# AugmentariumLab/VolumeRenderer

Measured on AMD Instinct MI355X. Metric: Mvoxels/s kd-tree compress+decode, higher is better.
Workload: dtype u8; 1 GPU; 2048x2048x1920 uint8 volume per GPU as 960 bricks of 256x256x128, rm_volume, tolerance 1, maxEpochs 2, VolumeKdtree build + levelCut

## Files before the change

volumerenderer_amd/csrc/brickset.h:

```cpp
#pragma once
#include "kd_common.h"
#include "../../include/vrhip.h"
#include <algorithm>
#include <string>
#include <vector>

namespace vr {

struct Stream2 {
    uint8_t *temp = nullptr;
    uint8_t *codes = nullptr;
    uint8_t *recon[3] = {nullptr, nullptr, nullptr};
    Ctrl *ctrl = nullptr;
    uint8_t *tree = nullptr;
    uint8_t *treeCompact = nullptr;
};

#define EST_R0_BUDGET 8
struct Switches {
    bool decodeWalk = false;
    bool decodeFineV1 = false;
    bool decodeQuad = false;
    bool noSkipBlocks = false;
    bool noUniformBlocks = false;
    bool estExactBounds = false;
    int estBudget = EST_R0_BUDGET;
    bool pyramidBoxes = false;
    bool indexPerBlock = false;
    bool noUniformDecode = false;
};

#define VR_LOD_SLOTS 4
struct LodSlot {
    int32_t *dev = nullptr;
    int32_t *host = nullptr;
    uint8_t *idxValCut = nullptr;
    uint32_t *decTables = nullptr;
    uint8_t *rankVals = nullptr;
    int64_t *obDev = nullptr;
    int64_t *obHost = nullptr;
    vr_pool_entry *tabHost = nullptr;
    int64_t tabCap = 0;
    hipEvent_t done = nullptr;
    bool pending = false;
};

struct BrickSet {
    int32_t B = 0;
    Switches sw;
    Geom g{};
    TilePlan tile{};
    RegionPlan region{};
    Pyr12Plan pyr12{};
    int32_t D = 0, maxDepth = 0;
    int32_t tolerance = 6, maxEpochs = 5, variant = 0;
    int32_t K = 0;
    int32_t Ds = 0;
    int64_t heapStride = 0;
    int64_t leafStride = 0;
    int64_t codeStride = 0;
    int64_t reconStride = 0;
    bool leafless = false;
    int64_t treeCap = 0;
    int64_t nIdx = 0;

    Stream2 mid, rng;
    uint8_t *mmMin[2] = {nullptr, nullptr}, *mmMax[2] = {nullptr, nullptr};
    unsigned long long *blockErr = nullptr;
    int64_t nErrBlk = 0;
    void *estSumm = nullptr;
    int64_t estSummStride = 0;
    unsigned long long *blockL1 = nullptr;
    uint8_t *blockFlag = nullptr;
    uint8_t *blockFlagR = nullptr;
    uint8_t *blockAlive = nullptr, *blockVal = nullptr;
    unsigned long long *blockSpine = nullptr, *blockSpineR = nullptr;
    uint32_t *chainLut = nullptr;
    uint32_t *blockTot = nullptr, *blockOff = nullptr;
    bool idx64 = false;
    unsigned long long *blockOff64 = nullptr, *idxBase = nullptr;
    int64_t nEmitBlk = 0;
// ... 80 lines not shown
```

volumerenderer_amd/csrc/capi.hip:

```cpp
#include "../../include/vrhip.h"
#include "brickset.h"
#include "raymarch.h"
#include <math.h>
#include <stdio.h>
#include <stdlib.h>
#include <string.h>
#include <algorithm>
#include <array>
#include <atomic>
#include <map>
#include <mutex>
#include <new>

using namespace vr;

struct vr_brickset { BrickSet s; };

#define HIPCHK(x) do { hipError_t e_ = (x); if (e_ != hipSuccess) return e_ == hipErrorOutOfMemory ? VR_ERR_OOM : VR_ERR_NO_DEVICE; } while (0)

static bool device_ok()
{
    int n = 0;
    hipError_t e = hipGetDeviceCount(&n);
    if ((e != hipSuccess || n <= 0) && getenv("VRHIP_DEBUG"))
// ... 160 lines not shown
    const vr_status rc = alloc_encoder_buffers(b);
    if (rc != VR_OK) { (void)hipGetLastError(); free_encoder_buffers(b); return rc; }
    b.encoderReady = true;
    return VR_OK;
}

vr_status vr_brickset_destroy(vr_brickset *h)
{
    if (!h) return VR_OK;
    BrickSet &b = h->s;
    free_lod_slots(&b);
    hipFree(b.errTable);
    free_encoder_buffers(b);
    free_stream2(b.mid);
    free_stream2(b.rng);
    hipFree(b.brickOff); hipFree(b.compactOverflow);
    hipFree(b.idxOff); hipFree(b.idxVal); hipFree(b.idxValCut); hipFree(b.fineIdx); hipFree(b.idxVal3); hipFree(b.boxUniform); hipFree(b.chainTab); hipFree(b.decTables); hipFree(b.lut); hipFree(b.spread); hipFree(b.srcIdx); hipFree(b.ownerRank); hipFree(b.ownerSurv); hipFree(b.rankVals);
    for (int i = 0; i < 8; ++i) if (b.ev[i]) hipEventDestroy(b.ev[i]);
    if (b.evFork) hipEventDestroy(b.evFork);
    for (int i = 0; i < 3; ++i) { if (b.evJoinN[i]) hipEventDestroy(b.evJoinN[i]); if (b.auxN[i]) hipStreamDestroy(b.auxN[i]); }
    delete h;
    return VR_OK;
}

static bool pow2(int64_t v) { return v > 0 && (v & (v - 1)) == 0; }

static bool misaligned16(const void *p) { return ((uintptr_t)p & 15) != 0; }

vr_status vr_brickset_create(vr_brickset **out, int32_t num_bricks, const int64_t dims[3], int32_t tolerance,
                             int32_t max_epochs, int32_t variant)
{
    if (!out || !dims || num_bricks <= 0) return VR_ERR_INVALID;
    if (tolerance < 0 || max_epochs < 0 || variant < 0 || variant > 2) return VR_ERR_INVALID;
    for (int k = 0; k < 3; ++k) if (dims[k] <= 0) return VR_ERR_INVALID;
    if (max_epochs > VR_MAX_EPOCHS) return VR_ERR_UNSUPPORTED;
    bool general = !pow2(dims[0]) || !pow2(dims[1]) || !pow2(dims[2]) || dims[0] > 1024 || dims[1] > 1024 || dims[2] > 1024;
    if (dims[0] > (1ll << 20) || dims[1] > (1ll << 20) || dims[2] > (1ll << 20) || dims[0] * dims[1] * dims[2] >= (1ll << 32))
        return VR_ERR_UNSUPPORTED;
    if (!device_ok()) return VR_ERR_NO_DEVICE;
    vr_brickset *h = new (std::nothrow) vr_brickset();
    if (!h) return VR_ERR_OOM;
    BrickSet &b = h->s;
    b.B = num_bricks;
    {
        Switches &w = b.sw;
        w.decodeWalk = getenv("VRHIP_DECODE_WALK") != nullptr;
        w.decodeFineV1 = getenv("VRHIP_DECODE_FINE_V1") != nullptr;
        w.decodeQuad = getenv("VRHIP_DECODE_QUAD") != nullptr;
        w.noSkipBlocks = getenv("VRHIP_NO_SKIP_BLOCKS") != nullptr;
        w.noUniformBlocks = getenv("VRHIP_NO_UNIFORM_BLOCKS") != nullptr;
        w.noUniformDecode = getenv("VRHIP_NO_UNIFORM_DECODE") != nullptr;
        w.pyramidBoxes = getenv("VRHIP_PYRAMID_BOXES") != nullptr;
        w.indexPerBlock = getenv("VRHIP_INDEX_PER_BLOCK") != nullptr;
        w.estExactBounds = getenv("VRHIP_EST_EXACT_BOUNDS") != nullptr;
        if (const char *eb = getenv("VRHIP_EST_BUDGET")) { const int v = atoi(eb); if (v >= 0) w.estBudget = v; }
    }
    make_geom(b.g, dims);
    b.D = b.g.D;
    if (b.D > 31) { delete h; return VR_ERR_UNSUPPORTED; }
    b.idx64 = b.D > 28 || (getenv("VRHIP_FORCE_IDX64") && b.D >= 12);
    if (b.idx64) general = true;
    if (b.idx64 && num_bricks != 1 && b.D > 28) { delete h; return VR_ERR_UNSUPPORTED; }
    b.generalGeom = general;
    b.maxDepth = b.D + VR_CHAIN_LEVELS;
    b.tolerance = tolerance; b.maxEpochs = max_epochs; b.variant = variant;
    b.K = b.D < 6 ? b.D : 6;
    b.Ds = b.D - b.K;
    b.heapStride = (int64_t)1 << (b.D + 1);
    b.leafStride = (int64_t)1 << b.D;
    b.codeStride = ((b.heapStride + 15) / 16) * 4;
    b.reconStride = b.leafStride;
    const int64_t numMax = b.heapStride - 1 + VR_CHAIN_LEVELS * b.leafStride;
    b.treeCap = ((numMax + 15) / 16 + 2) * 4 + 256;
    if (b.D >= 12) {
        const int64_t gappedBytes = ((int64_t)1 << (b.D - 12)) * 2320 * 4 + 256;
        if (gappedBytes > b.treeCap) b.treeCap = gappedBytes;
    }
    b.nIdx = (int64_t)1 << b.Ds;
    make_plans(b.g, b.K, b.generalGeom, b.idx64, b.treeCap, b.tile, b.region, b.pyr12);
    vr_status rc = alloc_stream2(b, b.mid);
    if (rc == VR_OK) {
        hipError_t e = hipMalloc(&b.idxOff, (size_t)b.B * b.nIdx * sizeof(uint32_t));
        if (e == hipSuccess) e = hipMalloc(&b.idxVal, (size_t)b.B * b.nIdx);
        if (e == hipSuccess) e = hipMalloc(&b.idxValCut, (size_t)b.B * b.nIdx);
        if (e == hipSuccess && general) {
            const int grc = build_general_geometry(&b);
            if (grc != 0) e = grc == -3 ? hipErrorOutOfMemory : hipErrorUnknown;
        }
        const auto upload = [](uint32_t *dst, const std::vector<uint32_t> &v) {
            return hipMemcpy(dst, v.data(), v.size() * sizeof(uint32_t), hipMemcpyHostToDevice);
        };
        if (e == hipSuccess) e = hipMalloc(&b.lut, ((size_t)1 << b.K) * sizeof(uint32_t));
        if (e == hipSuccess && !general) e = upload(b.lut, make_lut(b.g, b.K));
        if (e == hipSuccess && !general) e = hipMalloc(&b.spread, (size_t)(b.g.X + b.g.Y + b.g.Z) * sizeof(uint32_t));
        if (e == hipSuccess && !general) e = upload(b.spread, make_spread(b.g));
        for (int i = 0; i < 8 && e == hipSuccess; ++i) e = hipEventCreate(&b.ev[i]);
        if (e != hipSuccess) rc = e == hipErrorOutOfMemory ? VR_ERR_OOM : VR_ERR_NO_DEVICE;
    }
    if (rc != VR_OK) { vr_brickset_destroy(h); return rc; }
    b.hostCtrl.resize(b.B);
    b.openTreeBytes.assign(b.B, -1);
    *out = h;
    return VR_OK;
}

vr_status vr_brickset_set_switch(vr_brickset *h, const char *name, int32_t value)
{
    if (!h || !name) return VR_ERR_INVALID;
    Switches &w = h->s.sw;
    const bool on = value != 0;
    if (!strcmp(name, "decode_walk")) w.decodeWalk = on;
    else if (!strcmp(name, "decode_fine_v1")) w.decodeFineV1 = on;
    else if (!strcmp(name, "decode_quad")) w.decodeQuad = on;
    else if (!strcmp(name, "no_skip_blocks")) w.noSkipBlocks = on;
    else if (!strcmp(name, "no_uniform_blocks")) w.noUniformBlocks = on;
    else if (!strcmp(name, "no_uniform_decode")) w.noUniformDecode = on;
    else if (!strcmp(name, "pyramid_boxes")) w.pyramidBoxes = on;
    else if (!strcmp(name, "index_per_block")) w.indexPerBlock = on;
    else if (!strcmp(name, "est_exact_bounds")) w.estExactBounds = on;
    else return VR_ERR_INVALID;
    return VR_OK;
}

vr_status vr_brickset_set_compaction(vr_brickset *h, int32_t on_build)
{
    if (!h) return VR_ERR_INVALID;
    h->s.compactOnBuild = on_build != 0;
    return VR_OK;
}

vr_status vr_debug_set(const char *name, int32_t value)
{
    if (!name) return VR_ERR_INVALID;
    if (!strcmp(name, "skip_grid_v1")) { vr::g_skipGridV1.store(value ? 1 : 0); return VR_OK; }
    if (!strcmp(name, "reslice_tile_w")) {
        if (value != 8 && value != 16 && value != 64) return VR_ERR_INVALID;
        vr::g_resliceTileLog2.store(value == 8 ? 3 : (value == 16 ? 4 : 6));
        return VR_OK;
    }
    if (!strcmp(name, "hist_plain")) { vr::g_histPlain.store(value ? 1 : 0); return VR_OK; }
    return VR_ERR_INVALID;
}

vr_status vr_brickset_set_error_tolerance(vr_brickset *h, int32_t tol)
{
    if (!h || tol < 0) return VR_ERR_INVALID;
    h->s.tolerance = tol;
    return VR_OK;
}
vr_status vr_brickset_set_max_epochs(vr_brickset *h, int32_t e)
{
    if (!h || e < 0) return VR_ERR_INVALID;
    if (e > VR_MAX_EPOCHS) return VR_ERR_UNSUPPORTED;
    h->s.maxEpochs = e;
    return VR_OK;
}

vr_status vr_brickset_build(vr_brickset *h, const uint8_t *vox, void *stream)
{
    if (!h || !vox) return VR_ERR_INVALID;
    BrickSet &b = h->s;
    if (build_loads_vectors(&b) && misaligned16(vox)) return VR_ERR_INVALID;
    if (b.encoderReady && b.leafless != leafless_build(b)) {
        HIPCHK(hipDeviceSynchronize());
        free_encoder_buffers(b);
    }
    vr_status rc = ensure_encoder_buffers(b);
    if (rc != VR_OK) return rc;
    b.hostCtrlValid = false;
    b.hostBrickOff.clear();
    b.foreign = false;
// ... 1059 lines not shown
```

volumerenderer_amd/csrc/kd_encode.hip:

```cpp
#include "brickset.h"
#include <math.h>
#include <stdio.h>
#include <stdlib.h>
#include <string.h>

namespace vr {

#define FILL_NODES_PER_BLOCK 1024
#define EMIT_RANKS_PER_BLOCK 256

template <bool FROM_VOXELS>
__global__ void __launch_bounds__(256)
k_pyramid(Geom g, int dLeaf, int L, const uint8_t *__restrict__ vox, const uint8_t *__restrict__ inMin,
          const uint8_t *__restrict__ inMax, int64_t inStride, uint8_t *__restrict__ temp, int64_t heapStride,
          uint8_t *__restrict__ tempRange, uint8_t *__restrict__ outMin, uint8_t *__restrict__ outMax,
          int64_t outStride, const uint32_t *__restrict__ srcIdx)
{
    __shared__ uint8_t smn[2][1024], smx[2][1024];
    const int brick = blockIdx.y;
    const uint32_t n = 1u << L;
    const uint32_t base = blockIdx.x << L;
    uint8_t *T = temp + (int64_t)brick * heapStride;
    uint8_t *TR = tempRange ? tempRange + (int64_t)brick * heapStride : nullptr;
    for (uint32_t i = threadIdx.x; i < n; i += blockDim.x) {
// ... 2439 lines not shown
            if (b < nb && deadS[b]) { const uint32_t v4 = (uint32_t)valS[b] * 0x01010101u; pVal[t] = make_uint4(v4, v4, v4, v4); }
        }
#pragma unroll
        for (int k = 0; k < IDX_BLOCKS / 8; ++k) {
            const uint32_t p = (uint32_t)t + 256u * k, b = p >> 5;
            if (b < nb && deadS[b]) { const uint32_t v4 = (uint32_t)valS[b] * 0x01010101u; pVal3[p] = make_uint4(v4, v4, v4, v4); }
        }
    }
    if (w >= nLive) return;
    int dist[10];
#pragma unroll
    for (int i = 0; i < 10; ++i) dist[i] = __builtin_amdgcn_readfirstlane((int)distS[i]);
    if (D == 12) dist[0] = 0;
    const auto entry = [&](const IdxLoads &L, uint32_t b) {
        const uint32_t blk = blk0 + b;
        int val = idx_step(valS[b], rootS[b], dist[0]);
        uint32_t code6 = 0;
#pragma unroll
        for (int q = 1; q < 7; ++q) {
            code6 = L.cb[q] >> ((idx_off(idx_first(D, blk, q), lane, q) & 3u) * 2u);
            val = idx_step(val, code6, dist[q]);
        }
        const uint32_t c5 = L.c5 >> ((lane & 1u) * 4u);
        const bool root3 = (code6 & 3u) == 3u;
        const int64_t io = io0 + ((int64_t)blk << 6) + lane;
        a.idxOff[io] = (L.local != VR_IDX_DEAD && !root3) ? (a.idxBase ? 0u : blk * (uint32_t)PE_TOKENS) + L.local : VR_IDX_DEAD;
        a.idxVal[io] = (uint8_t)val;
        int v5[2], v4[4];
        uint32_t lo3 = 0, hi3 = 0;
#pragma unroll
        for (int i = 0; i < 2; ++i) v5[i] = idx_step(val, c5 >> (2 * i), dist[7]);
#pragma unroll
        for (int i = 0; i < 4; ++i) v4[i] = idx_step(v5[i >> 1], L.c4 >> (2 * i), dist[8]);
#pragma unroll
        for (int i = 0; i < 8; ++i) {
            const uint32_t v = (uint32_t)idx_step(v4[i >> 1], L.c3 >> (2 * i), dist[9]);
            if (i < 4) lo3 |= v << (8 * i); else hi3 |= v << (8 * (i - 4));
        }
        *(uint2 *)(a.idxVal3 + io * 8) = make_uint2(lo3, hi3);
    };
    const auto block_of = [&](uint32_t e) { return (uint32_t)__builtin_amdgcn_readfirstlane((int)listS[e]); };
    for (uint32_t e = w; e < nLive; e += 8u) {
        const uint32_t e1 = e + 4u < nLive ? e + 4u : e;
        const IdxLoads oth = idx_loads(a, Cb, io0, blk0 + block_of(e1), lane);
        entry(cur, block_of(e));
        if (e1 == e) break;
        const uint32_t e2 = e + 8u < nLive ? e + 8u : e1;
        cur = idx_loads(a, Cb, io0, blk0 + block_of(e2), lane);
        entry(oth, block_of(e1));
    }
}

#define CC_BLOCKS 16
#define CC_BATCH 4
template <bool RANGE>
__global__ void __launch_bounds__(256)
k_concat12(EmitArgs a, const uint8_t *__restrict__ gap, int64_t nblk)
{
    __shared__ unsigned long long g0S[CC_BLOCKS], spineS[CC_BLOCKS];
    __shared__ uint32_t totS[CC_BLOCKS], cntS[CC_BLOCKS];
    __shared__ unsigned long long bwIdx[2 * CC_BLOCKS];
    __shared__ uint32_t bwVal[2 * CC_BLOCKS];
    __shared__ uint32_t chunkPre[CC_BLOCKS + 1];
    __shared__ uint8_t chunkBlk[CC_BLOCKS * (PE_WORDS / 4 + 4)];
    const int brick = blockIdx.y, t = threadIdx.x;
    Ctrl &c = a.ctrls[brick];
    if (c.constBrick) return;
    if (a.brickOff && a.brickOff[gridDim.y] > (unsigned long long)a.compactCap) return;
    const int64_t blk0 = (int64_t)blockIdx.x * CC_BLOCKS;
    const int64_t base = a.brickOff ? (int64_t)a.brickOff[brick] : (int64_t)brick * a.treeCap;
    uint32_t *G0 = (uint32_t *)((RANGE ? a.treeR : a.tree) + base);
    const uint64_t capTok = a.brickOff ? ~0ull >> 2 : (uint64_t)a.treeCap * 4ull;
    if (t < 2 * CC_BLOCKS) { bwIdx[t] = ~0ull; bwVal[t] = 0u; }
    if (t < CC_BLOCKS) {
        const int64_t blk = blk0 + t;
        unsigned long long g0 = 0, sp = 0;
        uint32_t tot = 0, cnt = 0;
        if (blk < nblk) {
            const int64_t bo = (int64_t)brick * a.nEmitBlk + blk;
            const int bflags = a.blockAlive[bo];
            sp = RANGE ? a.blockSpineR[bo] : a.blockSpine[bo];
            g0 = a.blockOff64 ? a.blockOff64[bo] : (unsigned long long)a.blockOff[bo];
            tot = (bflags & 1) ? a.blockTot[bo] : 0u;
            cnt = (bflags & 2) && tot ? tot - (uint32_t)(sp >> 56) : 0u;
            if (tot && g0 + tot + 32ull > capTok) { atomicMax(&c.emitOverflow, 1); tot = 0; cnt = 0; }
        }
        g0S[t] = g0; spineS[t] = sp; totS[t] = tot; cntS[t] = cnt;
    }
    __syncthreads();
    if (t < CC_BLOCKS && totS[t] != 0u && totS[t] <= 32u) {
        const unsigned long long g0 = g0S[t];
        const uint32_t tot = totS[t], cnt = cntS[t];
        const int nsp = (int)(spineS[t] >> 56);
        unsigned long long v = spineS[t] & 0x00FFFFFFFFFFFFFFull;
        if (cnt) {
            const uint32_t *slot = (const uint32_t *)(gap + (int64_t)brick * a.treeCap) + (size_t)(blk0 + t) * PE_WORDS;
            unsigned long long sv = slot[0];
            if (cnt > 16u) sv |= (unsigned long long)slot[1] << 32;
            if (cnt < 32u) sv &= (1ull << (2 * cnt)) - 1ull;
            v |= sv << (2 * nsp);
        }
        const uint32_t sh = (uint32_t)(g0 & 15ull) * 2u;
        const uint64_t w0 = g0 >> 4, wl = (g0 + tot - 1) >> 4;
        const uint32_t x0 = (uint32_t)(v << sh), x1 = (uint32_t)((v << sh) >> 32), x2 = sh ? (uint32_t)(v >> (64u - sh)) : 0u;
        bwIdx[2 * t] = w0; bwVal[2 * t] = x0;
        if (wl == w0 + 1) { bwIdx[2 * t + 1] = wl; bwVal[2 * t + 1] = x1; }
        else if (wl == w0 + 2) { G0[w0 + 1] = x1; bwIdx[2 * t + 1] = wl; bwVal[2 * t + 1] = x2; }
    }
    if (t == 0) {
        uint32_t run = 0;
        for (int i = 0; i < CC_BLOCKS; ++i) {
            chunkPre[i] = run;
            if (totS[i] > 32u) {
                const uint64_t w0 = g0S[i] >> 4, wl = (g0S[i] + totS[i] - 1) >> 4;
                run += (uint32_t)((wl - (w0 & ~3ull)) / 4 + 1);
            }
        }
        chunkPre[CC_BLOCKS] = run;
    }
    __syncthreads();
    const uint32_t nchunkAll = chunkPre[CC_BLOCKS];
    for (int i = 0; i < CC_BLOCKS; ++i)
        for (uint32_t j = chunkPre[i] + (uint32_t)t; j < chunkPre[i + 1]; j += 256u) chunkBlk[j] = (uint8_t)i;
    __syncthreads();
    const uint32_t *gapW = (const uint32_t *)(gap + (int64_t)brick * a.treeCap) + (size_t)blk0 * PE_WORDS;
    for (uint32_t j0 = (uint32_t)t; j0 < nchunkAll; j0 += 256u * CC_BATCH) {
        uint32_t sv[CC_BATCH][5];
#pragma unroll
        for (int k = 0; k < CC_BATCH; ++k) {
            const uint32_t j = j0 + 256u * (uint32_t)k;
#pragma unroll
            for (int m = 0; m < 5; ++m) sv[k][m] = 0u;
            if (j >= nchunkAll) continue;
            const int i = chunkBlk[j];
            const unsigned long long g0 = g0S[i];
            const uint32_t cnt = cntS[i];
            const int nsp = (int)(spineS[i] >> 56);
            const int nws = (int)((cnt + 15u) >> 4);
            const uint32_t *slot = gapW + (size_t)i * PE_WORDS;
            const uint64_t wA = (g0 >> 4) & ~3ull;
            const long long so = 2ll * ((long long)(16ull * wA) - (long long)g0 - nsp) + 128ll * (long long)(j - chunkPre[i]);
            const int sw = (int)(so >> 5);
            if (cnt && sw >= 0 && sw + 4 < nws) {
                struct __attribute__((packed, aligned(4))) U4 { uint32_t x, y, z, w; };
                const U4 u = *(const U4 *)(slot + sw);
                sv[k][0] = u.x; sv[k][1] = u.y; sv[k][2] = u.z; sv[k][3] = u.w; sv[k][4] = slot[sw + 4];
            } else {
#pragma unroll
                for (int m = 0; m < 5; ++m) sv[k][m] = (cnt && sw + m >= 0 && sw + m < nws) ? slot[sw + m] : 0u;
            }
        }
#pragma unroll
        for (int k = 0; k < CC_BATCH; ++k) {
            const uint32_t j = j0 + 256u * (uint32_t)k;
            if (j >= nchunkAll) continue;
            const int i = chunkBlk[j];
            const unsigned long long g0 = g0S[i];
            const uint32_t tot = totS[i], cnt = cntS[i];
            const int nsp = (int)(spineS[i] >> 56);
            const unsigned long long spine = spineS[i] & 0x00FFFFFFFFFFFFFFull;
            const uint64_t w0 = g0 >> 4, wl = (g0 + tot - 1) >> 4;
            const uint64_t wA = w0 & ~3ull;
            const uint32_t q = j - chunkPre[i];
            const uint64_t d0 = wA + 4ull * (uint64_t)q;
            const long long so = 2ll * ((long long)(16ull * wA) - (long long)g0 - nsp) + 128ll * (long long)q;
            const uint32_t shf = (uint32_t)(so & 31ll);
            uint32_t o[4];
            const int tok0 = (int)(so >> 1);
            const bool edge = tok0 < 0 || tok0 + 64 > (int)cnt;
#pragma unroll
            for (int m = 0; m < 4; ++m) {
                o[m] = __builtin_amdgcn_alignbit(sv[k][m + 1], sv[k][m], shf);
                if (edge) {
                    const int tokAt = tok0 + 16 * m;
                    if (tokAt + 16 > (int)cnt) {
                        const int keep = (int)cnt - tokAt;
                        o[m] = keep <= 0 ? 0u : (keep >= 16 ? o[m] : (o[m] & ((1u << (2 * keep)) - 1u)));
                    }
                    if (tokAt < 0 && nsp) {
                        const long long bo2 = 2ll * ((long long)(16ull * (d0 + m)) - (long long)g0);
                        o[m] |= bo2 >= 0 ? (bo2 < 64 ? (uint32_t)(spine >> bo2) : 0u) : (uint32_t)(spine << (-bo2));
                    }
                }
            }
            if (d0 > w0 && d0 + 3 < wl) {
                *(uint4 *)(G0 + d0) = make_uint4(o[0], o[1], o[2], o[3]);
            } else {
#pragma unroll
                for (int m = 0; m < 4; ++m) {
                    const uint64_t d = d0 + m;
                    if (d < w0 || d > wl) continue;
                    if (d == w0) { bwIdx[2 * i] = d; bwVal[2 * i] = o[m]; }
                    else if (d == wl) { bwIdx[2 * i + 1] = d; bwVal[2 * i + 1] = o[m]; }
                    else G0[d] = o[m];
                }
            }
        }
    }
    __syncthreads();
    if (t < 2 * CC_BLOCKS) {
        const unsigned long long w = bwIdx[t];
        if (w != ~0ull) {
            bool first = true;
            uint32_t v = 0;
            unsigned long long wFirst = ~0ull, wLast = 0;
            for (int j = 0; j < 2 * CC_BLOCKS; ++j) {
                const unsigned long long wj = bwIdx[j];
                if (wj == ~0ull) continue;
                if (wFirst == ~0ull) wFirst = wj;
                wLast = wj;
                if (wj == w) { v |= bwVal[j]; if (j < t) first = false; }
            }
            if (first) {
                if (w == wFirst || w == wLast) { if (v) atomicOr(&G0[w], v); }
                else G0[w] = v;
            }
        }
    }
}

__global__ void __launch_bounds__(1024)
k_emit_stats(EmitArgs a, int64_t nblk)
{
    __shared__ unsigned long long sh[16];
    const int brick = blockIdx.x;
    if (a.ctrls[brick].constBrick) return;
    unsigned long long v = 0;
    for (int64_t i = threadIdx.x; i < nblk; i += blockDim.x) v = stat_merge(v, a.blockL1[(int64_t)brick * a.nEmitBlk + i]);
    for (int o = 32; o > 0; o >>= 1) v = stat_merge(v, __shfl_xor(v, o));
    if ((threadIdx.x & 63) == 0) sh[threadIdx.x >> 6] = v;
    __syncthreads();
    if (threadIdx.x == 0) {
        unsigned long long t = 0;
        for (int i = 0; i < 16; ++i) t = stat_merge(t, sh[i]);
        Ctrl &c = a.ctrls[brick];
        c.statL1 = t & ((1ull << 40) - 1ull);
        c.maxErrBefore = (int)((t >> 40) & 255ull);
        c.maxErrAfter = (int)((t >> 48) & 255ull);
    }
}

__global__ void __launch_bounds__(256)
k_const_finish(int D, Ctrl *ctrls, uint8_t *tree, int64_t treeCap, uint32_t *idxOff, uint8_t *idxVal, int64_t nIdx,
               const unsigned long long *brickOff = nullptr, int64_t compactCap = 0)
{
    const int brick = blockIdx.y;
    Ctrl &c = ctrls[brick];
    if (!c.constBrick) return;
    if (brickOff && brickOff[gridDim.y] > (unsigned long long)compactCap) return;
    const int v = c.constVal;
    if (blockIdx.x == 0 && threadIdx.x == 0) {
        for (int d = 0; d <= D; ++d) c.distanceMap[d] = d == 0 ? (uint8_t)v : 0;
        c.numActive = v ? 3 : 1;
        *(uint32_t *)(tree + (brickOff ? (int64_t)brickOff[brick] : (int64_t)brick * treeCap)) = v ? 0x3Du : 0x03u;
        c.numReverts = 0; c.maxErrBefore = 0; c.maxErrAfter = 0; c.statL1 = 0; c.emitOverflow = 0;
    }
    const int64_t s = (int64_t)blockIdx.x * 256 + threadIdx.x;
    if (s < nIdx) {
        idxOff[(int64_t)brick * nIdx + s] = VR_IDX_DEAD;
        idxVal[(int64_t)brick * nIdx + s] = (uint8_t)v;
    }
}

__global__ void k_const_finish_range(int D, Ctrl *ctrlsR, uint8_t *treeR, int64_t treeCap, const unsigned long long *brickOff = nullptr,
                                     int64_t compactCap = 0)
{
    Ctrl &c = ctrlsR[blockIdx.x];
    if (threadIdx.x || !c.constBrick) return;
    if (brickOff && brickOff[gridDim.x] > (unsigned long long)compactCap) return;
    const int v = c.constVal;
    for (int d = 0; d <= D; ++d) c.distanceMap[d] = 0;
// ... 72 lines not shown
    }
}

static bool dbg_sync(hipStream_t st, const char *phase)
{
    static const bool on = getenv("VRHIP_SYNC") != nullptr;
    if (!on) return true;
    hipError_t e = hipStreamSynchronize(st);
    fprintf(stderr, "[vrhip] phase %s: %s\n", phase, hipGetErrorString(e));
    return e == hipSuccess;
}

static void fill_emit_args(BrickSet *bs, EmitArgs &a)
{
    const bool mr = bs->variant == 2;
    a.codes = bs->mid.codes; a.codesR = mr ? bs->rng.codes : nullptr;
    a.temp = bs->mid.temp; a.tempR = mr ? bs->rng.temp : nullptr;
    a.rb = ReconBufs{{bs->mid.recon[0], bs->mid.recon[1], bs->mid.recon[2]}};
    a.rbR = ReconBufs{{bs->rng.recon[0], bs->rng.recon[1], bs->rng.recon[2]}};
    a.ctrls = bs->mid.ctrl; a.ctrlsR = mr ? bs->rng.ctrl : nullptr;
    a.heapStride = bs->heapStride; a.leafStride = bs->reconStride; a.codeStride = bs->codeStride;
    a.D = bs->D; a.maxDepth = bs->maxDepth; a.tol = kernel_tolerance(*bs); a.Ds = bs->Ds; a.K = bs->K;
    a.blockTot = bs->blockTot; a.blockOff = bs->blockOff; a.nEmitBlk = bs->nEmitBlk;
    a.blockOff64 = bs->blockOff64; a.idxBase = bs->idxBase;
    a.blockL1 = bs->blockL1;
    a.blockAlive = bs->blockAlive; a.blockVal = bs->blockVal; a.blockSpine = bs->blockSpine; a.blockSpineR = bs->blockSpineR;
    a.tree = bs->mid.tree; a.treeR = mr ? bs->rng.tree : nullptr; a.treeCap = bs->treeCap;
    a.brickOff = nullptr; a.compactCap = 0;
    a.idxOff = bs->idxOff; a.idxVal = bs->idxVal; a.idxVal3 = bs->idxVal3; a.nIdx = bs->nIdx;
    a.chainLut = bs->chainLut;
}

int compact_launch(BrickSet *bs, hipStream_t st)
{
    const int D = bs->D, B = bs->B;
    const bool mr = bs->variant == 2;
    if (!bs->brickOff && hipMalloc(&bs->brickOff, (size_t)(B + 1) * sizeof(unsigned long long)) != hipSuccess) return -3;
    if (!bs->compactOverflow && hipMalloc(&bs->compactOverflow, sizeof(int32_t)) != hipSuccess) return -3;
    if (bs->compactCap == 0) {
        int64_t cap = (int64_t)B * bs->g.voxels / 8 * 5 + (int64_t)B * 64 + 4096;
        const int64_t worst = (int64_t)B * bs->treeCap;
        if (cap > worst) cap = worst;
        if (hipMalloc(&bs->mid.treeCompact, (size_t)cap) != hipSuccess) return -3;
        if (mr && hipMalloc(&bs->rng.treeCompact, (size_t)cap) != hipSuccess) { hipFree(bs->mid.treeCompact); bs->mid.treeCompact = nullptr; return -3; }
        bs->compactCap = cap;
    }
    EmitArgs a;
    fill_emit_args(bs, a);
    a.tree = bs->mid.treeCompact; a.treeR = mr ? bs->rng.treeCompact : nullptr;
    a.brickOff = bs->brickOff; a.compactCap = bs->compactCap;
    const int64_t nblk = cdiv((int64_t)1 << D, 4096);
    hipLaunchKernelGGL(k_brick_offsets, dim3(1), dim3(1024), 0, st, bs->mid.ctrl, B, bs->brickOff, bs->compactCap, bs->compactOverflow);
    hipLaunchKernelGGL(k_emit_zero, dim3(cdiv(nblk, 256), B), dim3(256), 0, st, a, nblk);
    hipLaunchKernelGGL(k_concat12<false>, dim3(cdiv(nblk, CC_BLOCKS), B), dim3(256), 0, st, a, bs->mid.tree, nblk);
    if (mr) hipLaunchKernelGGL(k_concat12<true>, dim3(cdiv(nblk, CC_BLOCKS), B), dim3(256), 0, st, a, bs->rng.tree, nblk);
    hipLaunchKernelGGL(k_const_finish, dim3(1, B), dim3(64), 0, st, D, bs->mid.ctrl, bs->mid.treeCompact,
                       bs->treeCap, bs->idxOff, bs->idxVal, (int64_t)0, bs->brickOff, bs->compactCap);
    if (mr) hipLaunchKernelGGL(k_const_finish_range, dim3(B), dim3(64), 0, st, D, bs->rng.ctrl, bs->rng.treeCompact, bs->treeCap, bs->brickOff, bs->compactCap);
    bs->compactValid = true;
    return launch_status("compact");
}

static int ensure_aux(BrickSet *bs, int n)
{
    if (n > 3) n = 3;
    if (!bs->evFork && hipEventCreateWithFlags(&bs->evFork, hipEventDisableTiming) != hipSuccess) return 0;
    int have = 0;
    for (int i = 0; i < n; ++i) {
        if (!bs->auxN[i] && hipStreamCreateWithFlags(&bs->auxN[i], hipStreamNonBlocking) != hipSuccess) break;
        if (!bs->evJoinN[i] && hipEventCreateWithFlags(&bs->evJoinN[i], hipEventDisableTiming) != hipSuccess) break;
        ++have;
    }
    bs->aux = bs->auxN[0]; bs->evJoin = bs->evJoinN[0];
    return have;
}

int encode_launch(BrickSet *bs, const uint8_t *vox, hipStream_t st)
{
    const int D = bs->D, B = bs->B;
    const bool mr = bs->variant == 2;
    hipEventRecord(bs->ev[0], st);
    const uint8_t *rootMinP = nullptr, *rootMaxP = nullptr;
    const bool fused = D >= 12;
    if (bs->leafless != leafless_build(*bs)) return -2;
    bool skipOn = fused && bs->blockFlag && (!mr || bs->blockFlagR) && bs->tolerance >= 1 && bs->maxEpochs >= 1 && D >= 14 && !bs->sw.noSkipBlocks;
    const int64_t rootStride = (int64_t)1 << (D > 10 ? D - 10 : 0);
    {
        int dLeaf = D, round = 0;
        const uint8_t *inMin = nullptr, *inMax = nullptr;
        int64_t inStride = 0;
        const int64_t oStride = (int64_t)1 << (D > 10 ? D - 10 : 0);
        const Pyr12Plan &pp = bs->pyr12;
        skipOn = skipOn && pp.use12;
        if (pp.use12) {
            Pyr12Geom pg{};
            pg.ax = pp.ax; pg.ay = pp.ay; pg.az = pp.az;
            memcpy(pg.sx, pp.sx, sizeof(pg.sx));
            pg.swz = pp.swz; pg.nbx = pp.nbx; pg.nby = pp.nby; pg.lnbx = pp.lnbx; pg.lnby = pp.lnby;
            pg.spread = bs->spread;
            if (pp.lines && !bs->sw.pyramidBoxes)
                hipLaunchKernelGGL(k_pyramid12_lines, dim3((unsigned)((int64_t)1 << (D - 15)), B), dim3(256), 0, st, bs->g, pg, vox,
                                   bs->mid.temp, bs->heapStride, mr ? bs->rng.temp : nullptr, bs->mmMin[0], bs->mmMax[0],
                                   oStride, skipOn ? bs->blockFlag : nullptr, skipOn && mr ? bs->blockFlagR : nullptr);
            else
                hipLaunchKernelGGL(k_pyramid12, dim3((unsigned)((int64_t)1 << (D - 12)), B), dim3(256), 0, st, bs->g, pg, vox,
                                   bs->mid.temp, bs->heapStride, mr ? bs->rng.temp : nullptr, bs->mmMin[0], bs->mmMax[0],
                                   oStride, skipOn ? bs->blockFlag : nullptr, skipOn && mr ? bs->blockFlagR : nullptr);
            dLeaf = D - 12;
// ... 140 lines not shown
```

Baseline: 301,800 Mvoxels/s.

## Restructure compaction concat kernel into per-wavefront row processing with precomputed interiors

Replaces the per-thread chunk loop in the tree-compaction concat kernel with a row-based scheme. Each wavefront handles 64-chunk rows of one block, using wave-uniform metadata read through readfirstlane and a precomputed interior chunk range. That lets interior chunks do unconditional vector loads and stores, and edge chunks go through a separate slow path. The old kernel is kept behind a switch, and block metadata and short-block and boundary handling are factored into helpers. It also adds an overflow check on the token count. The goal is less per-chunk branching and divergence, at the cost of more shared-memory bookkeeping and tail imbalance across rows.

```diff
diff --git a/volumerenderer_amd/csrc/brickset.h b/volumerenderer_amd/csrc/brickset.h
--- a/volumerenderer_amd/csrc/brickset.h
+++ b/volumerenderer_amd/csrc/brickset.h
@@ -27,6 +27,7 @@
     int estBudget = EST_R0_BUDGET;
     bool pyramidBoxes = false;
     bool indexPerBlock = false;
+    bool concatChunks = false;
     bool noUniformDecode = false;
 };
 
diff --git a/volumerenderer_amd/csrc/capi.hip b/volumerenderer_amd/csrc/capi.hip
--- a/volumerenderer_amd/csrc/capi.hip
+++ b/volumerenderer_amd/csrc/capi.hip
@@ -236,6 +236,7 @@
         w.noUniformDecode = getenv("VRHIP_NO_UNIFORM_DECODE") != nullptr;
         w.pyramidBoxes = getenv("VRHIP_PYRAMID_BOXES") != nullptr;
         w.indexPerBlock = getenv("VRHIP_INDEX_PER_BLOCK") != nullptr;
+        w.concatChunks = getenv("VRHIP_CONCAT_CHUNKS") != nullptr;
         w.estExactBounds = getenv("VRHIP_EST_EXACT_BOUNDS") != nullptr;
         if (const char *eb = getenv("VRHIP_EST_BUDGET")) { const int v = atoi(eb); if (v >= 0) w.estBudget = v; }
     }
@@ -301,6 +302,7 @@
     else if (!strcmp(name, "no_uniform_decode")) w.noUniformDecode = on;
     else if (!strcmp(name, "pyramid_boxes")) w.pyramidBoxes = on;
     else if (!strcmp(name, "index_per_block")) w.indexPerBlock = on;
+    else if (!strcmp(name, "concat_chunks")) w.concatChunks = on;
     else if (!strcmp(name, "est_exact_bounds")) w.estExactBounds = on;
     else return VR_ERR_INVALID;
     return VR_OK;
diff --git a/volumerenderer_amd/csrc/kd_encode.hip b/volumerenderer_amd/csrc/kd_encode.hip
--- a/volumerenderer_amd/csrc/kd_encode.hip
+++ b/volumerenderer_amd/csrc/kd_encode.hip
@@ -2515,10 +2515,132 @@
 }
 
 #define CC_BLOCKS 16
-#define CC_BATCH 4
+#define CC_CHUNK_BATCH 4
+
+struct CcBlock {
+    unsigned long long g0, spine;
+    uint32_t tot, cnt;
+    int nsp;
+    const uint32_t *slot;
+};
+
+__device__ __forceinline__ long long cc_bit_offset(const CcBlock &b, uint32_t q)
+{
+    const uint64_t wA = (b.g0 >> 4) & ~3ull;
+    return 2ll * ((long long)(16ull * wA) - (long long)b.g0 - b.nsp) + 128ll * (long long)q;
+}
+
+__device__ __forceinline__ void cc_chunk_load(const CcBlock &b, uint32_t q, uint32_t sv[5])
+{
+    const int nws = (int)((b.cnt + 15u) >> 4);
+    const int sw = (int)(cc_bit_offset(b, q) >> 5);
+    if (b.cnt && sw >= 0 && sw + 4 < nws) {
+        struct __attribute__((packed, aligned(4))) U4 { uint32_t x, y, z, w; };
+        const U4 u = *(const U4 *)(b.slot + sw);
+        sv[0] = u.x; sv[1] = u.y; sv[2] = u.z; sv[3] = u.w; sv[4] = b.slot[sw + 4];
+    } else {
+#pragma unroll
+        for (int m = 0; m < 5; ++m) sv[m] = (b.cnt && sw + m >= 0 && sw + m < nws) ? b.slot[sw + m] : 0u;
+    }
+}
+
+__device__ __forceinline__ void cc_chunk_store(const CcBlock &b, uint32_t q, const uint32_t sv[5], uint32_t *G0,
+                                               unsigned long long *bw0, uint32_t *bv0)
+{
+    const uint64_t w0 = b.g0 >> 4, wl = (b.g0 + b.tot - 1) >> 4;
+    const uint64_t wA = w0 & ~3ull;
+    const uint64_t d0 = wA + 4ull * (uint64_t)q;
+    const long long so = cc_bit_offset(b, q);
+    const uint32_t shf = (uint32_t)(so & 31ll);
+    uint32_t o[4];
+    const int tok0 = (int)(so >> 1);
+    const bool edge = tok0 < 0 || tok0 + 64 > (int)b.cnt;
+#pragma unroll
+    for (int m = 0; m < 4; ++m) {
+        o[m] = __builtin_amdgcn_alignbit(sv[m + 1], sv[m], shf);
+        if (edge) {
+            const int tokAt = tok0 + 16 * m;
+            if (tokAt + 16 > (int)b.cnt) {
+                const int keep = (int)b.cnt - tokAt;
+                o[m] = keep <= 0 ? 0u : (keep >= 16 ? o[m] : (o[m] & ((1u << (2 * keep)) - 1u)));
+            }
+            if (tokAt < 0 && b.nsp) {
+                const long long bo2 = 2ll * ((long long)(16ull * (d0 + m)) - (long long)b.g0);
+                o[m] |= bo2 >= 0 ? (bo2 < 64 ? (uint32_t)(b.spine >> bo2) : 0u) : (uint32_t)(b.spine << (-bo2));
+            }
+        }
+    }
+    if (d0 > w0 && d0 + 3 < wl) {
+        *(uint4 *)(G0 + d0) = make_uint4(o[0], o[1], o[2], o[3]);
+    } else {
+#pragma unroll
+        for (int m = 0; m < 4; ++m) {
+            const uint64_t d = d0 + m;
+            if (d < w0 || d > wl) continue;
+            if (d == w0) { bw0[0] = d; bv0[0] = o[m]; }
+            else if (d == wl) { bw0[1] = d; bv0[1] = o[m]; }
+            else G0[d] = o[m];
+        }
+    }
+}
+
+__device__ __forceinline__ void cc_short_block(unsigned long long g0, unsigned long long sp, uint32_t tot, uint32_t cnt,
+                                               const uint32_t *slot, uint32_t *G0, unsigned long long *bw0, uint32_t *bv0)
+{
+    const int nsp = (int)(sp >> 56);
+    unsigned long long v = sp & 0x00FFFFFFFFFFFFFFull;
+    if (cnt) {
+        unsigned long long sv = slot[0];
+        if (cnt > 16u) sv |= (unsigned long long)slot[1] << 32;
+        if (cnt < 32u) sv &= (1ull << (2 * cnt)) - 1ull;
+        v |= sv << (2 * nsp);
+    }
+    const uint32_t sh = (uint32_t)(g0 & 15ull) * 2u;
+    const uint64_t w0 = g0 >> 4, wl = (g0 + tot - 1) >> 4;
+    const uint32_t x0 = (uint32_t)(v << sh), x1 = (uint32_t)((v << sh) >> 32), x2 = sh ? (uint32_t)(v >> (64u - sh)) : 0u;
+    bw0[0] = w0; bv0[0] = x0;
+    if (wl == w0 + 1) { bw0[1] = wl; bv0[1] = x1; }
+    else if (wl == w0 + 2) { G0[w0 + 1] = x1; bw0[1] = wl; bv0[1] = x2; }
+}
+
+__device__ __forceinline__ void cc_boundary_words(int t, const unsigned long long *bwIdx, const uint32_t *bwVal, uint32_t *G0)
+{
+    if (t >= 2 * CC_BLOCKS) return;
+    const unsigned long long w = bwIdx[t];
+    if (w == ~0ull) return;
+    bool first = true;
+    uint32_t v = 0;
+    unsigned long long wFirst = ~0ull, wLast = 0;
+    for (int j = 0; j < 2 * CC_BLOCKS; ++j) {
+        const unsigned long long wj = bwIdx[j];
+        if (wj == ~0ull) continue;
+        if (wFirst == ~0ull) wFirst = wj;
+        wLast = wj;
+        if (wj == w) { v |= bwVal[j]; if (j < t) first = false; }
+    }
+    if (first) {
+        if (w == wFirst || w == wLast) { if (v) atomicOr(&G0[w], v); }
+        else G0[w] = v;
+    }
+}
+
+__device__ __forceinline__ void cc_block_meta(const EmitArgs &a, bool range, Ctrl &c, int brick, int64_t blk, int64_t nblk, uint64_t capTok,
+                                              unsigned long long &g0, unsigned long long &sp, uint32_t &tot, uint32_t &cnt)
+{
+    g0 = 0; sp = 0; tot = 0; cnt = 0;
+    if (blk >= nblk) return;
+    const int64_t bo = (int64_t)brick * a.nEmitBlk + blk;
+    const int bflags = a.blockAlive[bo];
+    sp = range ? a.blockSpineR[bo] : a.blockSpine[bo];
+    g0 = a.blockOff64 ? a.blockOff64[bo] : (unsigned long long)a.blockOff[bo];
+    tot = (bflags & 1) ? a.blockTot[bo] : 0u;
+    cnt = (bflags & 2) && tot ? tot - (uint32_t)(sp >> 56) : 0u;
+    if (tot && (g0 + tot + 32ull > capTok || tot > (uint32_t)PE_TOKENS)) { atomicMax(&c.emitOverflow, 1); tot = 0; cnt = 0; }
+}
+
 template <bool RANGE>
 __global__ void __launch_bounds__(256)
-k_concat12(EmitArgs a, const uint8_t *__restrict__ gap, int64_t nblk)
+k_concat12_chunks(EmitArgs a, const uint8_t *__restrict__ gap, int64_t nblk)
 {
     __shared__ unsigned long long g0S[CC_BLOCKS], spineS[CC_BLOCKS];
     __shared__ uint32_t totS[CC_BLOCKS], cntS[CC_BLOCKS];
@@ -2536,40 +2658,15 @@
     const uint64_t capTok = a.brickOff ? ~0ull >> 2 : (uint64_t)a.treeCap * 4ull;
     if (t < 2 * CC_BLOCKS) { bwIdx[t] = ~0ull; bwVal[t] = 0u; }
     if (t < CC_BLOCKS) {
-        const int64_t blk = blk0 + t;
-        unsigned long long g0 = 0, sp = 0;
-        uint32_t tot = 0, cnt = 0;
-        if (blk < nblk) {
-            const int64_t bo = (int64_t)brick * a.nEmitBlk + blk;
-            const int bflags = a.blockAlive[bo];
-            sp = RANGE ? a.blockSpineR[bo] : a.blockSpine[bo];
-            g0 = a.blockOff64 ? a.blockOff64[bo] : (unsigned long long)a.blockOff[bo];
-            tot = (bflags & 1) ? a.blockTot[bo] : 0u;
-            cnt = (bflags & 2) && tot ? tot - (uint32_t)(sp >> 56) : 0u;
-            if (tot && g0 + tot + 32ull > capTok) { atomicMax(&c.emitOverflow, 1); tot = 0; cnt = 0; }
-        }
+        unsigned long long g0, sp;
+        uint32_t tot, cnt;
+        cc_block_meta(a, RANGE, c, brick, blk0 + t, nblk, capTok, g0, sp, tot, cnt);
         g0S[t] = g0; spineS[t] = sp; totS[t] = tot; cntS[t] = cnt;
     }
     __syncthreads();
-    if (t < CC_BLOCKS && totS[t] != 0u && totS[t] <= 32u) {
-        const unsigned long long g0 = g0S[t];
-        const uint32_t tot = totS[t], cnt = cntS[t];
-        const int nsp = (int)(spineS[t] >> 56);
-        unsigned long long v = spineS[t] & 0x00FFFFFFFFFFFFFFull;
-        if (cnt) {
-            const uint32_t *slot = (const uint32_t *)(gap + (int64_t)brick * a.treeCap) + (size_t)(blk0 + t) * PE_WORDS;
-            unsigned long long sv = slot[0];
-            if (cnt > 16u) sv |= (unsigned long long)slot[1] << 32;
-            if (cnt < 32u) sv &= (1ull << (2 * cnt)) - 1ull;
-            v |= sv << (2 * nsp);
-        }
-        const uint32_t sh = (uint32_t)(g0 & 15ull) * 2u;
-        const uint64_t w0 = g0 >> 4, wl = (g0 + tot - 1) >> 4;
-        const uint32_t x0 = (uint32_t)(v << sh), x1 = (uint32_t)((v << sh) >> 32), x2 = sh ? (uint32_t)(v >> (64u - sh)) : 0u;
-        bwIdx[2 * t] = w0; bwVal[2 * t] = x0;
-        if (wl == w0 + 1) { bwIdx[2 * t + 1] = wl; bwVal[2 * t + 1] = x1; }
-        else if (wl == w0 + 2) { G0[w0 + 1] = x1; bwIdx[2 * t + 1] = wl; bwVal[2 * t + 1] = x2; }
-    }
+    const uint32_t *gapW = (const uint32_t *)(gap + (int64_t)brick * a.treeCap) + (size_t)blk0 * PE_WORDS;
+    if (t < CC_BLOCKS && totS[t] != 0u && totS[t] <= 32u)
+        cc_short_block(g0S[t], spineS[t], totS[t], cntS[t], gapW + (size_t)t * PE_WORDS, G0, &bwIdx[2 * t], &bwVal[2 * t]);
     if (t == 0) {
         uint32_t run = 0;
         for (int i = 0; i < CC_BLOCKS; ++i) {
@@ -2586,100 +2683,143 @@
     for (int i = 0; i < CC_BLOCKS; ++i)
         for (uint32_t j = chunkPre[i] + (uint32_t)t; j < chunkPre[i + 1]; j += 256u) chunkBlk[j] = (uint8_t)i;
     __syncthreads();
-    const uint32_t *gapW = (const uint32_t *)(gap + (int64_t)brick * a.treeCap) + (size_t)blk0 * PE_WORDS;
-    for (uint32_t j0 = (uint32_t)t; j0 < nchunkAll; j0 += 256u * CC_BATCH) {
-        uint32_t sv[CC_BATCH][5];
-#pragma unroll
-        for (int k = 0; k < CC_BATCH; ++k) {
+    const auto block_of = [&](uint32_t j) {
+        const int i = chunkBlk[j];
+        return CcBlock{g0S[i], spineS[i] & 0x00FFFFFFFFFFFFFFull, totS[i], cntS[i], (int)(spineS[i] >> 56), gapW + (size_t)i * PE_WORDS};
+    };
+    for (uint32_t j0 = (uint32_t)t; j0 < nchunkAll; j0 += 256u * CC_CHUNK_BATCH) {
+        uint32_t sv[CC_CHUNK_BATCH][5];
+#pragma unroll
+        for (int k = 0; k < CC_CHUNK_BATCH; ++k) {
             const uint32_t j = j0 + 256u * (uint32_t)k;
 #pragma unroll
             for (int m = 0; m < 5; ++m) sv[k][m] = 0u;
             if (j >= nchunkAll) continue;
-            const int i = chunkBlk[j];
-            const unsigned long long g0 = g0S[i];
-            const uint32_t cnt = cntS[i];
-            const int nsp = (int)(spineS[i] >> 56);
-            const int nws = (int)((cnt + 15u) >> 4);
-            const uint32_t *slot = gapW + (size_t)i * PE_WORDS;
-            const uint64_t wA = (g0 >> 4) & ~3ull;
-            const long long so = 2ll * ((long long)(16ull * wA) - (long long)g0 - nsp) + 128ll * (long long)(j - chunkPre[i]);
-            const int sw = (int)(so >> 5);
-            if (cnt && sw >= 0 && sw + 4 < nws) {
-                struct __attribute__((packed, aligned(4))) U4 { uint32_t x, y, z, w; };
-                const U4 u = *(const U4 *)(slot + sw);
-                sv[k][0] = u.x; sv[k][1] = u.y; sv[k][2] = u.z; sv[k][3] = u.w; sv[k][4] = slot[sw + 4];
-            } else {
-#pragma unroll
-                for (int m = 0; m < 5; ++m) sv[k][m] = (cnt && sw + m >= 0 && sw + m < nws) ? slot[sw + m] : 0u;
-            }
-        }
-#pragma unroll
-        for (int k = 0; k < CC_BATCH; ++k) {
+            cc_chunk_load(block_of(j), j - chunkPre[chunkBlk[j]], sv[k]);
+        }
+#pragma unroll
+        for (int k = 0; k < CC_CHUNK_BATCH; ++k) {
             const uint32_t j = j0 + 256u * (uint32_t)k;
             if (j >= nchunkAll) continue;
             const int i = chunkBlk[j];
-            const unsigned long long g0 = g0S[i];
-            const uint32_t tot = totS[i], cnt = cntS[i];
-            const int nsp = (int)(spineS[i] >> 56);
-            const unsigned long long spine = spineS[i] & 0x00FFFFFFFFFFFFFFull;
+            cc_chunk_store(block_of(j), j - chunkPre[i], sv[k], G0, &bwIdx[2 * i], &bwVal[2 * i]);
+        }
+    }
+    __syncthreads();
+    cc_boundary_words(t, bwIdx, bwVal, G0);
+}
+
+#define CC_ROW 64
+#ifndef CC_BATCH
+#define CC_BATCH 4
+#endif
+#define CC_MAX_ROWS (CC_BLOCKS * ((PE_WORDS / 4 + 4 + CC_ROW - 1) / CC_ROW))
+template <bool RANGE>
+__global__ void __launch_bounds__(256)
+k_concat12(EmitArgs a, const uint8_t *__restrict__ gap, int64_t nblk)
+{
+    __shared__ unsigned long long g0S[CC_BLOCKS], spineS[CC_BLOCKS];
+    __shared__ uint32_t totS[CC_BLOCKS], cntS[CC_BLOCKS];
+    __shared__ unsigned long long bwIdx[2 * CC_BLOCKS];
+    __shared__ uint32_t bwVal[2 * CC_BLOCKS];
+    __shared__ unsigned long long wAS[CC_BLOCKS];
+    __shared__ int sw0S[CC_BLOCKS], qi0S[CC_BLOCKS], qi1S[CC_BLOCKS];
+    __shared__ uint32_t shfS[CC_BLOCKS], nchS[CC_BLOCKS];
+    __shared__ uint32_t rowPre[CC_BLOCKS + 1];
+    __shared__ uint8_t rowBlk[CC_MAX_ROWS];
+    const int brick = blockIdx.y, t = threadIdx.x;
+    Ctrl &c = a.ctrls[brick];
+    if (c.constBrick) return;
+    if (a.brickOff && a.brickOff[gridDim.y] > (unsigned long long)a.compactCap) return;
+    const int64_t blk0 = (int64_t)blockIdx.x * CC_BLOCKS;
+    const int64_t base = a.brickOff ? (int64_t)a.brickOff[brick] : (int64_t)brick * a.treeCap;
+    uint32_t *G0 = (uint32_t *)((RANGE ? a.treeR : a.tree) + base);
+    const uint64_t capTok = a.brickOff ? ~0ull >> 2 : (uint64_t)a.treeCap * 4ull;
+    if (t < 2 * CC_BLOCKS) { bwIdx[t] = ~0ull; bwVal[t] = 0u; }
+    if (t < CC_BLOCKS) {
+        unsigned long long g0, sp;
+        uint32_t tot, cnt;
+        cc_block_meta(a, RANGE, c, brick, blk0 + t, nblk, capTok, g0, sp, tot, cnt);
+        g0S[t] = g0; spineS[t] = sp; totS[t] = tot; cntS[t] = cnt;
+        unsigned long long wA = 0;
+        uint32_t nch = 0, shf = 0;
+        int sw0 = 0, qi0 = 0, qi1 = -1;
+        if (tot > 32u) {
             const uint64_t w0 = g0 >> 4, wl = (g0 + tot - 1) >> 4;
-            const uint64_t wA = w0 & ~3ull;
-            const uint32_t q = j - chunkPre[i];
-            const uint64_t d0 = wA + 4ull * (uint64_t)q;
-            const long long so = 2ll * ((long long)(16ull * wA) - (long long)g0 - nsp) + 128ll * (long long)q;
-            const uint32_t shf = (uint32_t)(so & 31ll);
-            uint32_t o[4];
-            const int tok0 = (int)(so >> 1);
-            const bool edge = tok0 < 0 || tok0 + 64 > (int)cnt;
-#pragma unroll
-            for (int m = 0; m < 4; ++m) {
-                o[m] = __builtin_amdgcn_alignbit(sv[k][m + 1], sv[k][m], shf);
-                if (edge) {
-                    const int tokAt = tok0 + 16 * m;
-                    if (tokAt + 16 > (int)cnt) {
-                        const int keep = (int)cnt - tokAt;
-                        o[m] = keep <= 0 ? 0u : (keep >= 16 ? o[m] : (o[m] & ((1u << (2 * keep)) - 1u)));
-                    }
-                    if (tokAt < 0 && nsp) {
-                        const long long bo2 = 2ll * ((long long)(16ull * (d0 + m)) - (long long)g0);
-                        o[m] |= bo2 >= 0 ? (bo2 < 64 ? (uint32_t)(spine >> bo2) : 0u) : (uint32_t)(spine << (-bo2));
-                    }
-                }
-            }
-            if (d0 > w0 && d0 + 3 < wl) {
-                *(uint4 *)(G0 + d0) = make_uint4(o[0], o[1], o[2], o[3]);
-            } else {
-#pragma unroll
-                for (int m = 0; m < 4; ++m) {
-                    const uint64_t d = d0 + m;
-                    if (d < w0 || d > wl) continue;
-                    if (d == w0) { bwIdx[2 * i] = d; bwVal[2 * i] = o[m]; }
-                    else if (d == wl) { bwIdx[2 * i + 1] = d; bwVal[2 * i + 1] = o[m]; }
-                    else G0[d] = o[m];
-                }
-            }
-        }
+            wA = w0 & ~3ull;
+            const int dw = (int)(wl - wA);
+            nch = (uint32_t)dw / 4u + 1u;
+            const int nws = (int)((cnt + 15u) >> 4);
+            const long long so0 = 2ll * ((long long)(16ull * wA) - (long long)g0 - (long long)(sp >> 56));
+            sw0 = (int)(so0 >> 5);
+            shf = (uint32_t)(so0 & 31ll);
+            qi0 = max(1, (3 - sw0) >> 2);
+            qi1 = cnt ? min((dw - 4) >> 2, (nws - 5 - sw0) >> 2) : -1;
+            if (qi1 < qi0) { qi0 = (int)nch; qi1 = (int)nch - 1; }
+        }
+        wAS[t] = wA; sw0S[t] = sw0; qi0S[t] = qi0; qi1S[t] = qi1; shfS[t] = shf; nchS[t] = nch;
+        const uint32_t rows = (nch + (uint32_t)CC_ROW - 1u) / (uint32_t)CC_ROW;
+        uint32_t incl = rows;
+#pragma unroll
+        for (int o = 1; o < CC_BLOCKS; o <<= 1) { const uint32_t n = __shfl_up(incl, o); if (t >= o) incl += n; }
+        rowPre[t] = incl - rows;
+        if (t == CC_BLOCKS - 1) rowPre[CC_BLOCKS] = incl;
+        for (uint32_t k = 0; k < rows; ++k) rowBlk[incl - rows + k] = (uint8_t)t;
     }
     __syncthreads();
-    if (t < 2 * CC_BLOCKS) {
-        const unsigned long long w = bwIdx[t];
-        if (w != ~0ull) {
-            bool first = true;
-            uint32_t v = 0;
-            unsigned long long wFirst = ~0ull, wLast = 0;
-            for (int j = 0; j < 2 * CC_BLOCKS; ++j) {
-                const unsigned long long wj = bwIdx[j];
-                if (wj == ~0ull) continue;
-                if (wFirst == ~0ull) wFirst = wj;
-                wLast = wj;
-                if (wj == w) { v |= bwVal[j]; if (j < t) first = false; }
-            }
-            if (first) {
-                if (w == wFirst || w == wLast) { if (v) atomicOr(&G0[w], v); }
-                else G0[w] = v;
-            }
-        }
-    }
+    const uint32_t *gapW = (const uint32_t *)(gap + (int64_t)brick * a.treeCap) + (size_t)blk0 * PE_WORDS;
+    {
+        const int s = t - (256 - CC_BLOCKS);
+        if (s >= 0 && totS[s] != 0u && totS[s] <= 32u)
+            cc_short_block(g0S[s], spineS[s], totS[s], cntS[s], gapW + (size_t)s * PE_WORDS, G0, &bwIdx[2 * s], &bwVal[2 * s]);
+    }
+    const uint32_t w = (uint32_t)__builtin_amdgcn_readfirstlane(t >> 6), lane = (uint32_t)t & 63u;
+    const uint32_t nrows = rowPre[CC_BLOCKS];
+    struct __attribute__((packed, aligned(4))) U4 { uint32_t x, y, z, w; };
+    for (uint32_t r0 = w; r0 < nrows; r0 += 4u * CC_BATCH) {
+        U4 u[CC_BATCH];
+        uint32_t u4[CC_BATCH], shf[CC_BATCH];
+        uint4 *dst[CC_BATCH];
+        bool in[CC_BATCH];
+#pragma unroll
+        for (int k = 0; k < CC_BATCH; ++k) {
+            const bool valid = r0 + 4u * (uint32_t)k < nrows;
+            const uint32_t r = valid ? r0 + 4u * (uint32_t)k : r0;
+            const int i = __builtin_amdgcn_readfirstlane((int)rowBlk[r]);
+            const uint32_t q0 = (r - (uint32_t)__builtin_amdgcn_readfirstlane((int)rowPre[i])) * (uint32_t)CC_ROW;
+            const int sw0 = __builtin_amdgcn_readfirstlane(sw0S[i]);
+            const int qi0 = __builtin_amdgcn_readfirstlane(qi0S[i]), qi1 = __builtin_amdgcn_readfirstlane(qi1S[i]);
+            shf[k] = (uint32_t)__builtin_amdgcn_readfirstlane((int)shfS[i]);
+            const int q = (int)(q0 + lane);
+            in[k] = valid && q >= qi0 && q <= qi1;
+            const uint32_t *src = gapW + (size_t)i * PE_WORDS + (in[k] ? sw0 + 4 * q : 0);
+            dst[k] = (uint4 *)(G0 + wAS[i]) + q;
+            u[k] = *(const U4 *)src;
+            u4[k] = src[4];
+        }
+        __builtin_amdgcn_sched_barrier(0);
+#pragma unroll
+        for (int k = 0; k < CC_BATCH; ++k) {
+            asm volatile("" : "+v"(u[k].x), "+v"(u[k].y), "+v"(u[k].z), "+v"(u[k].w), "+v"(u4[k]));
+            const uint4 o = make_uint4(__builtin_amdgcn_alignbit(u[k].y, u[k].x, shf[k]), __builtin_amdgcn_alignbit(u[k].z, u[k].y, shf[k]),
+                                       __builtin_amdgcn_alignbit(u[k].w, u[k].z, shf[k]), __builtin_amdgcn_alignbit(u4[k], u[k].w, shf[k]));
+            if (in[k]) *dst[k] = o;
+        }
+    }
+    {
+        const int i = t >> 4;
+        const int nch = (int)nchS[i], qi0 = qi0S[i], qi1 = qi1S[i];
+        const int ne = qi0 + (nch - 1 - qi1);
+        for (int e = t & 15; e < ne; e += 16) {
+            const uint32_t q = (uint32_t)(e < qi0 ? e : qi1 + 1 + (e - qi0));
+            const CcBlock b{g0S[i], spineS[i] & 0x00FFFFFFFFFFFFFFull, totS[i], cntS[i], (int)(spineS[i] >> 56), gapW + (size_t)i * PE_WORDS};
+            uint32_t sv[5];
+            cc_chunk_load(b, q, sv);
+            cc_chunk_store(b, q, sv, G0, &bwIdx[2 * i], &bwVal[2 * i]);
+        }
+    }
+    __syncthreads();
+    cc_boundary_words(t, bwIdx, bwVal, G0);
 }
 
 __global__ void __launch_bounds__(1024)
@@ -2858,8 +2998,9 @@
     const int64_t nblk = cdiv((int64_t)1 << D, 4096);
     hipLaunchKernelGGL(k_brick_offsets, dim3(1), dim3(1024), 0, st, bs->mid.ctrl, B, bs->brickOff, bs->compactCap, bs->compactOverflow);
     hipLaunchKernelGGL(k_emit_zero, dim3(cdiv(nblk, 256), B), dim3(256), 0, st, a, nblk);
-    hipLaunchKernelGGL(k_concat12<false>, dim3(cdiv(nblk, CC_BLOCKS), B), dim3(256), 0, st, a, bs->mid.tree, nblk);
-    if (mr) hipLaunchKernelGGL(k_concat12<true>, dim3(cdiv(nblk, CC_BLOCKS), B), dim3(256), 0, st, a, bs->rng.tree, nblk);
+    const bool chunks = bs->sw.concatChunks;
+    hipLaunchKernelGGL(chunks ? k_concat12_chunks<false> : k_concat12<false>, dim3(cdiv(nblk, CC_BLOCKS), B), dim3(256), 0, st, a, bs->mid.tree, nblk);
+    if (mr) hipLaunchKernelGGL(chunks ? k_concat12_chunks<true> : k_concat12<true>, dim3(cdiv(nblk, CC_BLOCKS), B), dim3(256), 0, st, a, bs->rng.tree, nblk);
     hipLaunchKernelGGL(k_const_finish, dim3(1, B), dim3(64), 0, st, D, bs->mid.ctrl, bs->mid.treeCompact,
                        bs->treeCap, bs->idxOff, bs->idxVal, (int64_t)0, bs->brickOff, bs->compactCap);
     if (mr) hipLaunchKernelGGL(k_const_finish_range, dim3(B), dim3(64), 0, st, D, bs->rng.ctrl, bs->rng.treeCompact, bs->treeCap, bs->brickOff, bs->compactCap);
```

Result: no change. 302,100 Mvoxels/s (median of 5 runs) (+0.1%).
